# yuliangguo/OmniFusion

Measured on AMD Instinct MI355X. Metric: panoramas/sec at 512x1024 ERP, N=18 256^2 patches; equi2pers+pers2equi GB/s vs HBM peak, higher is better.
Workload: dtype f16x3 (fp16 hi/lo pairs, fp32 accumulate: fp32-class); 1 GPU; cfg2/cfg4 shard: 8 panoramas/GPU/step, 512x1024 ERP, fov 80, nrows 4 (18 patches); full single-pass spherical_fusion forward (confidence=True) at patch size 128 — the only size the reference network exists at (SURVEY 0.1); random-init weights (seed 42); inputs resident in HBM; resample pair at 18x256^2 reported in roofline_resample; per_gpu_batch=8, global_batch=8, parallelism=image-sharded x1, execution=3 forwards in flight per GPU on 3 streams (spherical_fusion.pipelined)

## Files before the change

### include/omnifusion.h

```cpp
#ifndef OMNIFUSION_H_
#define OMNIFUSION_H_

#include <stddef.h>
#include <stdint.h>

#ifdef __cplusplus
extern "C" {
#endif

#define OMNI_VERSION 200

enum omni_status {
    OMNI_OK = 0,
    OMNI_ERR_INVALID = 1,
    OMNI_ERR_HIP = 2,
    OMNI_ERR_UNSUPPORTED = 3
};

enum omni_layout { OMNI_LAYOUT_BCHWN = 0, OMNI_LAYOUT_BNCHW = 1, OMNI_LAYOUT_BNHWC = 2,
                   OMNI_LAYOUT_BCHNW = 3  };
enum omni_dtype { OMNI_F32 = 0, OMNI_F16 = 1 };

typedef void* omni_stream_t;
typedef struct omni_geometry omni_geometry_t;
// ... 61 lines not shown
int omni_gemm_rows_sh_f16x3(const void* x, const void* wt16r, const float* bias, const float* res, void* dst, int fmt,
                            int rows, int K, int N, int act, omni_stream_t stream);
int omni_gemm_rows_pack(const void* wt16, void* wt16r, int N, int K, omni_stream_t stream);
int omni_gemm_rows_ln_sh_f16x3(const float* x, const float* ln_weight, const float* ln_bias, float eps, const void* wt16r, const float* bias,
                               const float* res, void* dst, int fmt, int rows, int N, int act, omni_stream_t stream);
int omni_conv3x3_up2_sh_f16x3(const void* src, const void* wt16, const float* bias, void* dst, int fmt,
                              int M, int Hl, int Wl, int C, int Cout, int act, omni_stream_t stream);
size_t omni_up2_heads_scratch_bytes(int M, int P);
int omni_conv3x3_up2_heads_sh_f16x3(const void* src, const void* wt16, const float* bias, const void* heads_w16f, float bias_pred, float bias_weight,
                                    float* scratch, size_t scratch_bytes, float* out_a, float* out_c, int M, int P, int confidence, omni_stream_t stream);
int omni_conv3x3_up2_heads_sh_f16x1(const void* src, const void* wt16, const float* bias, const void* heads_w16f, float bias_pred, float bias_weight,
                                    float* scratch, size_t scratch_bytes, float* out_a, float* out_c, int M, int P, int confidence, omni_stream_t stream);
int omni_heads_pack_f16x3(const float* w_host, void* dst_host);
int omni_conv2d_sh_f16x3_post_ws(const void* src1, const void* src2, const void* wt16, const float* bias,
                                 const void* res, void* dst, int fmt, int M, int H, int W, int C1, int C2, int Cout,
                                 int KH, int KW, int stride, int pad, int act, int splitk, float* ws, size_t ws_bytes,
                                 const float* post, size_t post_elems, omni_stream_t stream);
int omni_wino_input_sh(const void* src, void* V, int M, int H, int W, int C, omni_stream_t stream);
int omni_conv3x3_wino_sh_f16x3(const void* V, const void* wt16, const float* bias, const void* res, void* dst, int fmt,
                               int M, int H, int W, int C, int Cout, int act, int splitk, float* ws, size_t ws_bytes, omni_stream_t stream);
int omni_sh_from_f32(const float* src, void* dst, size_t n, omni_stream_t stream);
int omni_sh_to_f32(const void* src, float* dst, size_t n, omni_stream_t stream);
int omni_sh_overflow(int* flag, int reset);
int omni_stem_f32(const float* src, const float* wt, const float* bias, float* dst, int M, int P, omni_stream_t stream);
int omni_maxpool3x3s2_f32(const float* src, float* dst, int M, int H, int W, int C, omni_stream_t stream);
int omni_upsample_bilinear_f32(const float* src, float* dst, int M, int H, int W, int C, int Ho, int Wo, omni_stream_t stream);
int omni_add_hw_f32(float* x, const float* y, int M, int HW, int C, omni_stream_t stream);
int omni_add_period_f32(float* x, const float* y, size_t total, size_t period, omni_stream_t stream);
int omni_stem_sh(const float* src, const float* wt, const float* bias, void* dst, int M, int P, omni_stream_t stream);
int omni_stem_sh_f16x3(const float* src, const void* wt16, const float* bias, void* dst, int M, int P, omni_stream_t stream);
int omni_stem_sh_f16x1(const float* src, const void* wt16, const float* bias, void* dst, int M, int P, omni_stream_t stream);
int omni_maxpool3x3s2_sh(const void* src, void* dst, int M, int H, int W, int C, omni_stream_t stream);
int omni_upsample_bilinear_sh(const void* src, void* dst, int M, int H, int W, int C, int Ho, int Wo, omni_stream_t stream);
int omni_add_hw_sh(void* x, const float* y, int M, int HW, int C, omni_stream_t stream);
int omni_add_period_sh(void* x, const float* y, size_t total, size_t period, omni_stream_t stream);
int omni_layernorm512_sh(const float* x, const float* g, const float* b, void* y, int rows, float eps, omni_stream_t stream);
int omni_gemm_rows_slices_sh_f16x3(const void* x, const void* wt16r, float* parts, int rows, int K, int N, int slices, omni_stream_t stream);
int omni_gemm_rows_ln_parts_sh_f16x3(const float* parts, int nparts, const float* pbias, const float* pres, float* xout,
                                     const float* ln_weight, const float* ln_bias, float eps, const void* wt16r, const float* bias,
                                     void* dst, int fmt, int rows, int N, int act, omni_stream_t stream);
int omni_splitk_reduce_ln512(const float* parts, int nparts, const float* bias, const float* res, float* tok, const float* ln_weight, const float* ln_bias,
                             float eps, void* y, int fmt, int rows, omni_stream_t stream);
int omni_gemm_sh_f16x3_ln512_ws(const void* x, const void* wt16, const float* bias, const float* res, float* tok, const float* ln_g, const float* ln_b,
                                float eps, void* y, int fmt, int rows, int K, int splitk, float* ws, size_t ws_bytes, omni_stream_t stream);
int omni_attention_qkv_sh(const float* qkv, void* out, int B, int N, omni_stream_t stream);
int omni_token_pack_f32(const float* d, const float* pos, float* tok, int M, int N, int HW, int C, omni_stream_t stream);
int omni_layernorm512_f32(const float* x, const float* g, const float* b, float* y, int rows, float eps, omni_stream_t stream);
int omni_attention_f32(const float* q, const float* kv, float* out, int B, int N, omni_stream_t stream);
int omni_heads_f32(const float* x, const float* w, float bias_pred, float bias_weight, float* out_a, float* out_c,
                   int M, int P, int confidence, omni_stream_t stream);
int omni_mlp_points_f32(const float* xyz, const float* depth, const float* w1, const float* b1, const float* w2,
                        const float* b2, float* out, int Mo, int N, int HW, omni_stream_t stream);

int omni_masked_median_f32(const float* x, const float* mask, size_t n, unsigned* ws, float* out, omni_stream_t stream);
int omni_depth_metrics_f32(float* pred, const float* gt, const float* mask, const float* scale_num, const float* scale_den,
                           size_t n, double* ws, float* out, omni_stream_t stream);

size_t omni_semantic_workspace_bytes(size_t npix);
int omni_semantic_step_f32(const float* logits, const int64_t* target, int B, int C, size_t HW, int64_t ignore_index, int K,
                           void* workspace, float* loss, int64_t* pred, int64_t* confusion, omni_stream_t stream);
int omni_semantic_grad_f32(const float* logits, const int64_t* target, int B, int C, size_t HW, int64_t ignore_index,
                           const void* workspace, const float* grad_out, float* grad_logits, omni_stream_t stream);
int omni_confusion_matrix_i64(const int64_t* pred, const int64_t* gt, size_t n, int K, int64_t* confusion, int64_t* n_bad,
                              omni_stream_t stream);

int omni_preprocess_rgb_u8(const unsigned char* src_hwc, float* dst_chw, int B, int Hs, int Ws, int H, int W, omni_stream_t stream);
// ... 67 lines not shown
```

### omnifusion_amd/_lib.py

```python
import ctypes
import os

_HERE = os.path.dirname(os.path.abspath(__file__))
LIB_PATH = os.environ.get("OMNI_LIB_VARIANT") or os.path.join(_HERE, "csrc", "libomnifusion_hip.so")
LIB_PATH_DEBUG = os.path.join(_HERE, "csrc", "libomnifusion_hip_dbg.so")

OMNI_OK, OMNI_ERR_INVALID, OMNI_ERR_HIP, OMNI_ERR_UNSUPPORTED = 0, 1, 2, 3
LAYOUT_BCHWN, LAYOUT_BNCHW, LAYOUT_BNHWC, LAYOUT_BCHNW = 0, 1, 2, 3
F32, F16 = 0, 1

_lib = None


class OmniLibraryMissing(ImportError):
    pass


EXPORTS = [
    "omni_version", "omni_last_error", "omni_set_option", "omni_get_option", "omni_num_patches", "omni_patch_centers",
    "omni_geometry_create", "omni_geometry_destroy", "omni_geometry_cache_clear", "omni_geometry_cache_size",
    "omni_equi2pers", "omni_equi2pers_aux", "omni_pers2equi", "omni_pers2equi_conf", "omni_patches_to_planar",
    "omni_equi2pers_g", "omni_pers2equi_g", "omni_equi2pers_bwd", "omni_pers2equi_bwd",
    "omni_conv2d_nhwc_f32", "omni_stem_f32", "omni_maxpool3x3s2_f32", "omni_upsample_bilinear_f32",
    "omni_add_hw_f32", "omni_add_period_f32", "omni_token_pack_f32", "omni_layernorm512_f32",
    "omni_attention_f32", "omni_heads_f32", "omni_mlp_points_f32",
    "omni_conv2d_nhwc_f16x3_ws", "omni_conv2d_sh_f16x3_ws", "omni_conv2d_sh_f16x3_post_ws", "omni_gemm_rows_sh_f16x3", "omni_gemm_rows_ln_sh_f16x3", "omni_gemm_rows_pack", "omni_conv3x3_up2_sh_f16x3", "omni_conv3x3_up2_heads_sh_f16x3", "omni_conv3x3_up2_heads_sh_f16x1", "omni_up2_heads_scratch_bytes", "omni_heads_pack_f16x3", "omni_sh_from_f32", "omni_sh_to_f32", "omni_sh_overflow",
    "omni_stem_sh", "omni_stem_sh_f16x3", "omni_stem_sh_f16x1", "omni_maxpool3x3s2_sh", "omni_upsample_bilinear_sh", "omni_add_hw_sh", "omni_add_period_sh", "omni_layernorm512_sh", "omni_gemm_sh_f16x3_ln512_ws", "omni_gemm_rows_slices_sh_f16x3", "omni_gemm_rows_ln_parts_sh_f16x3", "omni_splitk_reduce_ln512", "omni_wino_input_sh", "omni_conv3x3_wino_sh_f16x3", "omni_attention_qkv_sh",
    "omni_conv2d_splitk_plan", "omni_conv2d_nhwc_f32_ws",
    "omni_masked_median_f32", "omni_depth_metrics_f32",
    "omni_png_info", "omni_png_decode", "omni_png_decode_batch", "omni_zlib_inflate", "omni_png_checksums",
    "omni_preprocess_rgb_u8", "omni_preprocess_depth_u16", "omni_berhu_workspace_bytes", "omni_berhu_loss_f32", "omni_berhu_grad_f32",
    "omni_pointcloud_ply_f32",
    "omni_dibr_workspace_bytes", "omni_splat_render_f32", "omni_dibr_f32",
    "omni_splat_render_wt_f32", "omni_dibr_wt_f32", "omni_dibr_bwd_workspace_bytes", "omni_splat_render_bwd_f32", "omni_dibr_bwd_f32",
    "omni_ssim_f32", "omni_photometric_workspace_bytes", "omni_photometric_grad_scratch_bytes", "omni_photometric_loss_f32",
    "omni_photometric_grad_f32",
    "omni_freeview_rotations", "omni_freeview_equi2pers_f32", "omni_freeview_pers2equi_f32", "omni_freeview_merge_f32",
    "omni_freeview_bwd_workspace_bytes", "omni_freeview_equi2pers_bwd_f32", "omni_freeview_pers2equi_bwd_f32", "omni_freeview_merge_bwd_f32",
    "omni_semantic_workspace_bytes", "omni_semantic_step_f32", "omni_semantic_grad_f32", "omni_confusion_matrix_i64",
]


def load():
    global _lib
    if _lib is not None:
        return _lib
    if not os.path.exists(LIB_PATH):
        raise OmniLibraryMissing(
            f"{LIB_PATH} not found: build it with `python -m omnifusion_amd.build` "
            "(hipcc --offload-arch=gfx950).  There is no fallback path.")
    import torch
    lib = ctypes.CDLL(LIB_PATH)
    lib.omni_last_error.restype = ctypes.c_char_p
    lib.omni_version.restype = ctypes.c_int
    lib.omni_up2_heads_scratch_bytes.restype = ctypes.c_size_t
    lib.omni_dibr_workspace_bytes.restype = ctypes.c_size_t
    lib.omni_splat_render_f32.argtypes = [ctypes.c_void_p] * 3 + [ctypes.c_float] + [ctypes.c_void_p] * 2 + [ctypes.c_int] * 4 + [ctypes.c_void_p] * 2
    lib.omni_dibr_f32.argtypes = [ctypes.c_void_p] * 4 + [ctypes.c_int, ctypes.c_float, ctypes.c_int] + [ctypes.c_void_p] * 2 + \
        [ctypes.c_int] * 4 + [ctypes.c_void_p] * 2
    vp, ci, cf = ctypes.c_void_p, ctypes.c_int, ctypes.c_float
# ... 83 lines not shown
```

### omnifusion_amd/csrc/omni_net.hip

```cpp
#include "omni_internal.h"
#include "omni_sh.h"

namespace {
typedef float f4v __attribute__((ext_vector_type(4)));

template <bool SH>
__global__ __launch_bounds__(256) void stem_kernel(const float* __restrict__ src, const float* __restrict__ wt,
                                                   const float* __restrict__ bias, void* __restrict__ dst,
                                                   int M, int P, int Po)
{
    __shared__ __attribute__((aligned(16))) float wl[147 * 64];
    __shared__ float in[3][21][22];
    const int t = threadIdx.x;
    const int tiles = Po / 8;
    const int m = blockIdx.x / (tiles * tiles), tt = blockIdx.x % (tiles * tiles);
    const int oy0 = (tt / tiles) * 8, ox0 = (tt % tiles) * 8;
    for (int i = t; i < 147 * 64 / 4; i += 256) reinterpret_cast<f4v*>(wl)[i] = reinterpret_cast<const f4v*>(wt)[i];
    const int iy0 = oy0 * 2 - 3, ix0 = ox0 * 2 - 3;
    for (int i = t; i < 3 * 21 * 21; i += 256) {
        const int c = i / 441, r = (i % 441) / 21, q = i % 21;
        const int iy = iy0 + r, ix = ix0 + q;
        float v = 0.0f;
        if ((unsigned)iy < (unsigned)P && (unsigned)ix < (unsigned)P) v = src[((size_t)m * 3 + c) * P * P + (size_t)iy * P + ix];
        in[c][r][q] = v;
    }
    __syncthreads();
    const int p = t & 63, cg = (t >> 6) * 16;
    const int py = p >> 3, px = p & 7;
    float acc[16];
#pragma unroll
    for (int j = 0; j < 16; ++j) acc[j] = bias[cg + j];
    for (int ky = 0; ky < 7; ++ky)
// ... 81 lines not shown
    const int c8 = C / 8;
    const size_t total = (size_t)M * Ho * Wo * c8;
    if (i >= total) return;
    const int c = (int)(i % c8) * 8;
    size_t r = i / c8;
    const int ox = (int)(r % Wo); r /= Wo;
    const int oy = (int)(r % Ho); const int m = (int)(r / Ho);
    const float fy = fmaxf(sy * ((float)oy + 0.5f) - 0.5f, 0.0f), fx = fmaxf(sx * ((float)ox + 0.5f) - 0.5f, 0.0f);
    const int y0 = (int)fy, x0 = (int)fx;
    const int y1 = y0 + (y0 < H - 1 ? 1 : 0), x1 = x0 + (x0 < W - 1 ? 1 : 0);
    const float ly = fy - (float)y0, lx = fx - (float)x0, hy = 1.0f - ly, hx = 1.0f - lx;
    const size_t coff = (size_t)(c >> 5) * 128 + (c & 31) * 2;
    const size_t pp = (size_t)C * 4;
    const unsigned char* b = src + (size_t)m * H * W * pp + coff;
    const unsigned char* p00 = b + ((size_t)y0 * W + x0) * pp; const unsigned char* p01 = b + ((size_t)y0 * W + x1) * pp;
    const unsigned char* p10 = b + ((size_t)y1 * W + x0) * pp; const unsigned char* p11 = b + ((size_t)y1 * W + x1) * pp;
    const omni_h8v h00 = *reinterpret_cast<const omni_h8v*>(p00), l00 = *reinterpret_cast<const omni_h8v*>(p00 + 64);
    const omni_h8v h01 = *reinterpret_cast<const omni_h8v*>(p01), l01 = *reinterpret_cast<const omni_h8v*>(p01 + 64);
    const omni_h8v h10 = *reinterpret_cast<const omni_h8v*>(p10), l10 = *reinterpret_cast<const omni_h8v*>(p10 + 64);
    const omni_h8v h11 = *reinterpret_cast<const omni_h8v*>(p11), l11 = *reinterpret_cast<const omni_h8v*>(p11 + 64);
    omni_h8v oh, ol;
#pragma unroll
    for (int e = 0; e < 8; ++e) {
        const float v00 = fmaf((float)l00[e], 4.8828125e-4f, (float)h00[e]), v01 = fmaf((float)l01[e], 4.8828125e-4f, (float)h01[e]);
        const float v10 = fmaf((float)l10[e], 4.8828125e-4f, (float)h10[e]), v11 = fmaf((float)l11[e], 4.8828125e-4f, (float)h11[e]);
        const float o = hy * (hx * v00 + lx * v01) + ly * (hx * v10 + lx * v11);
        const _Float16 h = (fabsf(o) < 6.103515625e-05f) ? (_Float16)0.0f : (_Float16)o;
        oh[e] = h; ol[e] = (_Float16)((o - (float)h) * 2048.0f);
    }
    unsigned char* d = dst + (((size_t)m * Ho + oy) * Wo + ox) * pp + coff;
    *reinterpret_cast<omni_h8v*>(d) = oh; *reinterpret_cast<omni_h8v*>(d + 64) = ol;
}

__global__ __launch_bounds__(256) void add_hw_kernel(float* __restrict__ x, const float* __restrict__ y, size_t total, int HW, int C)
{
    const size_t i = (size_t)blockIdx.x * 256 + threadIdx.x;
    if (i >= total) return;
    const int c = (int)(i % C);
    const size_t m = i / ((size_t)HW * C);
    x[i] += y[m * C + c];
}
__global__ __launch_bounds__(256) void add_period_kernel(float* __restrict__ x, const float* __restrict__ y, size_t total, size_t period)
{
    const size_t i = (size_t)blockIdx.x * 256 + threadIdx.x;
    if (i >= total) return;
    x[i] += y[i % period];
}

__global__ __launch_bounds__(256) void add_hw_sh_kernel(void* __restrict__ x, const float* __restrict__ y, size_t total4, int HW, int C)
{
    const size_t i = (size_t)blockIdx.x * 256 + threadIdx.x;
    if (i >= total4) return;
    const size_t e = i * 4;
    const int c = (int)(e % C);
    const size_t m = e / ((size_t)HW * C);
    act_store4<true>(x, e, act_load4<true>(x, e) + *reinterpret_cast<const f4v*>(y + m * C + c));
}
__global__ __launch_bounds__(256) void add_period_sh_kernel(void* __restrict__ x, const float* __restrict__ y, size_t total4, size_t period)
{
    const size_t i = (size_t)blockIdx.x * 256 + threadIdx.x;
    if (i >= total4) return;
    const size_t e = i * 4;
    act_store4<true>(x, e, act_load4<true>(x, e) + *reinterpret_cast<const f4v*>(y + e % period));
}
__global__ __launch_bounds__(256) void token_pack_kernel(const float* __restrict__ d, const float* __restrict__ pos,
                                                         float* __restrict__ tok, int M, int N, int HW, int C)
// ... 201 lines not shown
}
int omni_add_hw_f32(float* x, const float* y, int M, int HW, int C, omni_stream_t stream)
{
    const size_t total = (size_t)M * HW * C;
    hipLaunchKernelGGL(add_hw_kernel, dim3(nblk(total)), dim3(256), 0, S_, x, y, total, HW, C);
    OMNI_HIP(hipGetLastError()); return OMNI_OK;
}
int omni_add_period_f32(float* x, const float* y, size_t total, size_t period, omni_stream_t stream)
{
    hipLaunchKernelGGL(add_period_kernel, dim3(nblk(total)), dim3(256), 0, S_, x, y, total, period);
    OMNI_HIP(hipGetLastError()); return OMNI_OK;
}
int omni_stem_sh(const float* src, const float* wt, const float* bias, void* dst, int M, int P, omni_stream_t stream)
{
    if (P % 16) OMNI_FAIL(OMNI_ERR_INVALID, "omni_stem: patch size must be a multiple of 16");
    const int Po = P / 2;
    hipLaunchKernelGGL(stem_kernel<true>, dim3(M * (Po / 8) * (Po / 8)), dim3(256), 0, S_, src, wt, bias, dst, M, P, Po);
    OMNI_HIP(hipGetLastError()); return OMNI_OK;
}
int omni_maxpool3x3s2_sh(const void* src, void* dst, int M, int H, int W, int C, omni_stream_t stream)
{
    if (C % 32) OMNI_FAIL(OMNI_ERR_INVALID, "SH tensors need C % 32 == 0");
    const int Ho = (H + 2 - 3) / 2 + 1, Wo = (W + 2 - 3) / 2 + 1;
    hipLaunchKernelGGL(maxpool_kernel<true>, dim3(nblk((size_t)M * Ho * Wo * C / 4)), dim3(256), 0, S_, src, dst, M, H, W, C, Ho, Wo);
    OMNI_HIP(hipGetLastError()); return OMNI_OK;
}
int omni_upsample_bilinear_sh(const void* src, void* dst, int M, int H, int W, int C, int Ho, int Wo, omni_stream_t stream)
{
    if (C % 32) OMNI_FAIL(OMNI_ERR_INVALID, "SH tensors need C % 32 == 0");
    hipLaunchKernelGGL(upsample_sh8_kernel, dim3(nblk((size_t)M * Ho * Wo * C / 8)), dim3(256), 0, S_, (const unsigned char*)src,
                       (unsigned char*)dst, M, H, W, C, Ho, Wo, (float)H / (float)Ho, (float)W / (float)Wo);
    OMNI_HIP(hipGetLastError()); return OMNI_OK;
}
int omni_add_hw_sh(void* x, const float* y, int M, int HW, int C, omni_stream_t stream)
{
    if (C % 32) OMNI_FAIL(OMNI_ERR_INVALID, "SH tensors need C % 32 == 0");
    const size_t total4 = (size_t)M * HW * C / 4;
    hipLaunchKernelGGL(add_hw_sh_kernel, dim3(nblk(total4)), dim3(256), 0, S_, x, y, total4, HW, C);
    OMNI_HIP(hipGetLastError()); return OMNI_OK;
}
int omni_add_period_sh(void* x, const float* y, size_t total, size_t period, omni_stream_t stream)
{
    if (total % 32 || period % 32) OMNI_FAIL(OMNI_ERR_INVALID, "SH tensors need C % 32 == 0");
    hipLaunchKernelGGL(add_period_sh_kernel, dim3(nblk(total / 4)), dim3(256), 0, S_, x, y, total / 4, period);
    OMNI_HIP(hipGetLastError()); return OMNI_OK;
}
int omni_layernorm512_sh(const float* x, const float* g, const float* b, void* y, int rows, float eps, omni_stream_t stream)
{
    hipLaunchKernelGGL(layernorm512_kernel<true>, dim3((rows + 3) / 4), dim3(256), 0, S_, x, g, b, y, rows, eps);
    OMNI_HIP(hipGetLastError()); return OMNI_OK;
}
int omni_attention_qkv_sh(const float* qkv, void* out, int B, int N, omni_stream_t stream)
{
    if (N > 64) OMNI_FAIL(OMNI_ERR_UNSUPPORTED, "omni_attention: at most 64 tokens");
    hipLaunchKernelGGL(attention_kernel<true>, dim3(B * 4, (N + 3) / 4), dim3(256), 0, S_, qkv, qkv + 512, out, N, 0.08838834764831845f, 1536, 1536, 512);
    OMNI_HIP(hipGetLastError()); return OMNI_OK;
}
int omni_token_pack_f32(const float* d, const float* pos, float* tok, int M, int N, int HW, int C, omni_stream_t stream)
{
    hipLaunchKernelGGL(token_pack_kernel, dim3(nblk((size_t)M * HW * C)), dim3(256), 0, S_, d, pos, tok, M, N, HW, C);
    OMNI_HIP(hipGetLastError()); return OMNI_OK;
}
int omni_layernorm512_f32(const float* x, const float* g, const float* b, float* y, int rows, float eps, omni_stream_t stream)
{
    hipLaunchKernelGGL(layernorm512_kernel<false>, dim3((rows + 3) / 4), dim3(256), 0, S_, x, g, b, (void*)y, rows, eps);
    OMNI_HIP(hipGetLastError()); return OMNI_OK;
// ... 23 lines not shown
```

### omnifusion_amd/model/_engine.py

```python
import ctypes
import os

import torch

from .. import _lib
from ..equi_pers.equi2pers_v3 import equi2pers_patches, equi2pers_aux, pair, _NPATCH
from ..equi_pers.pers2equi_v3 import pers2equi, pers2equi_conf

ACT_NONE, ACT_RELU, ACT_GELU = 0, 1, 2
_LAYERS = [("layer1", 3, 1), ("layer2", 4, 2), ("layer3", 6, 2), ("layer4", 3, 2)]
_BN_EPS = 1e-5
PRECISIONS = ("f16x3", "f16x1", "fp32")


def _p(t):
    return ctypes.c_void_p(t.data_ptr()) if t is not None else None


def split_weights_f16x3(w):
    w = w.to(torch.float32)
    wmax = float(w.abs().max()) if w.numel() else 0.0
    if not wmax < 65504.0:
        raise ValueError(f"folded weight magnitude {wmax:g} is outside the fp16 range of the f16x3 operand format: "
                         "run this checkpoint with OMNI_NET_PRECISION=fp32")
# ... 44 lines not shown
        g = sd[bn + ".weight"].double() / torch.sqrt(sd[bn + ".running_var"].double() + _BN_EPS)
        b = sd[bn + ".bias"].double() - sd[bn + ".running_mean"].double() * g
        return w * g[:, None, None, None], b

    @staticmethod
    def _gemm_layout(w):
        return w.permute(0, 2, 3, 1).reshape(w.shape[0], -1)

    def pack(self, state_dict, device):
        sd = {k: v.detach().cpu() for k, v in strip_module_prefix(state_dict).items()}
        dev = torch.device(device)
        f = lambda t: t.to(torch.float32).contiguous().to(dev)
        W = {}
        w, b = self._fold(sd, "conv1", "bn1")
        W["stem.w"] = f(w.permute(2, 3, 1, 0).reshape(147, 64)); W["stem.b"] = f(b)
        wk = torch.zeros((64, 3, 7, 8), dtype=torch.float64); wk[..., :7] = w
        W["stem.w16"] = split_weights_f16x3(torch.cat([wk.reshape(64, 168), torch.zeros((64, 24), dtype=torch.float64)], 1)).to(dev)

        def convbn(key, conv, bn):
            w, b = self._fold(sd, conv, bn)
            wg = self._gemm_layout(w).to(torch.float32)
            W[key + ".w"] = f(wg); W[key + ".b"] = f(b)
            W[key + ".w16"] = split_weights_f16x3(wg).to(dev)
        for lname, nblk, _ in _LAYERS:
            for i in range(nblk):
                p = f"{lname}.{i}"
                convbn(p + ".c1", p + ".conv1", p + ".bn1")
                convbn(p + ".c2", p + ".conv2", p + ".bn2")
                if (p + ".downsample.0.weight") in sd:
                    convbn(p + ".ds", p + ".downsample.0", p + ".downsample.1")
        for name in ("de_conv0_0", "de_conv0_1", "de_conv1_0", "de_conv1_1", "de_conv2_0", "de_conv2_1",
                     "de_conv3_0", "de_conv3_1", "de_conv4_0"):
            convbn(name, name + ".conv", name + ".bn")
        down = "down1" if self.iterative else "down"
        W["down.w"] = f(sd[down + ".weight"].reshape(32, 512)); W["down.b"] = f(sd[down + ".bias"])
        W["down.w16"] = split_weights_f16x3(sd[down + ".weight"].reshape(32, 512)).to(dev)
        W["pos"] = f(sd["transformer.pos_emb"].reshape(self.npatches, 512))
        for i in range(6):
            p = f"transformer.layer.{i}"
            for k in ("norm1.weight", "norm1.bias", "norm2.weight", "norm2.bias", "attn.q.weight", "attn.kv.weight",
                      "attn.proj.weight", "attn.proj.bias", "mlp.fc1.weight", "mlp.fc1.bias", "mlp.fc2.weight", "mlp.fc2.bias"):
                W[f"t{i}.{k}"] = f(sd[f"{p}.{k}"])
        for i in range(6):
            t = f"t{i}."
            W[t + "attn.qkv.w16"] = split_weights_f16x3(torch.cat([W[t + "attn.q.weight"], W[t + "attn.kv.weight"]], 0).cpu()).to(dev)
            for k in ("attn.proj", "mlp.fc1", "mlp.fc2"):
                W[t + k + ".w16"] = split_weights_f16x3(W[t + k + ".weight"].cpu()).to(dev)
        W["enc_norm.w"] = f(sd["transformer.encoder_norm.weight"]); W["enc_norm.b"] = f(sd["transformer.encoder_norm.bias"])
        hw = torch.stack([sd["pred.weight"][0, :, :, :, 0], sd["weight_pred.weight"][0, :, :, :, 0]])
        W["heads.w"] = f(hw.permute(0, 2, 3, 1).reshape(2, 9, 32))
        import numpy as np
        hw_host = np.ascontiguousarray(hw.permute(0, 2, 3, 1).reshape(2, 9, 32).to(torch.float32).numpy())
        frag = np.zeros(4 * 64 * 8, np.float16)
        _lib.check(_lib.load().omni_heads_pack_f16x3(hw_host.ctypes.data_as(ctypes.c_void_p), frag.ctypes.data_as(ctypes.c_void_p)), "heads_pack")
        W["heads.w16f"] = torch.from_numpy(frag).to(dev)
        self.head_bias = (float(sd["pred.bias"][0]), float(sd["weight_pred.bias"][0]))

        def mlp(name):
            w1, b1 = self._fold(sd, name + ".0", name + ".1")
            w2, b2 = self._fold(sd, name + ".3", name + ".4")
            return w1[:, :, 0, 0], b1, w2[:, :, 0, 0], b2
        P4 = self.patch_size[0] // 4
        if self.iterative:
            for name in ("mlp_points1", "mlp_points2"):
                w1, b1, w2, b2 = mlp(name)
                W[name + ".w1"], W[name + ".b1"], W[name + ".w2"], W[name + ".b2"] = f(w1), f(b1), f(w2), f(b2)
# ... 145 lines not shown
                                                      _p(self.w[bkey]) if bkey else None, None, _p(out), 1 if out_sh else 0, rows, Nout, act, self._s), "ln+gemm " + w16key)
            return out
        return self._gemm_sh(self._ln_sh(x, lnw, lnb, rows, eps), w16key, bkey, rows, 512, Nout, act=act, out_sh=out_sh)

    def _ln_sh(self, x, wk, bk, rows, eps):
        y = torch.empty_like(x)
        _lib.check(_lib.load().omni_layernorm512_sh(_p(x), _p(self.w[wk]), _p(self.w[bk]), _p(y), rows, ctypes.c_float(eps), self._s), "layernorm")
        return y

    def _ln(self, x, wk, bk, rows, eps):
        y = torch.empty_like(x)
        _lib.check(_lib.load().omni_layernorm512_f32(_p(x), _p(self.w[wk]), _p(self.w[bk]), _p(y), rows, ctypes.c_float(eps), self._s), "layernorm")
        return y

    def _up(self, x, M, H, Wd, C, Ho, Wo):
        y = torch.empty((M, Ho, Wo, C), dtype=torch.float32, device=x.device)
        fn = _lib.load().omni_upsample_bilinear_sh if self.sh else _lib.load().omni_upsample_bilinear_f32
        _lib.check(fn(_p(x), _p(y), M, H, Wd, C, Ho, Wo, self._s), "upsample")
        return y

    fold_point_feat = True
    fuse_up = True

    def _up_conv(self, x, key, M, H, Wd, C, Cout, act, out_f32=False, out=None):
        Ho, Wo = 2 * H, 2 * Wd
        if self.sh and self.fuse_up and Wo % 32 == 0 and Ho % 4 == 0:
            if out is None:
                out = torch.empty((M, Ho, Wo, Cout), dtype=torch.float32, device=x.device)
            _lib.check(_lib.load().omni_conv3x3_up2_sh_f16x3(_p(x), _p(self.w[key + ".w16"]), _p(self.w[key + ".b"]), _p(out),
                                                             (0 if out_f32 else 1) | (4 if (self._bs == 1 and self.latency_plan) else 0) | self._x1,
                                                             M, H, Wd, C, Cout, act, self._s), "up+conv " + key)
            return out
        return self._conv(self._up(x, M, H, Wd, C, Ho, Wo), key, M, Ho, Wo, C, Cout, 3, 1, 1, act, out_f32=out_f32, out=out)

    def transformer(self, d, bs):
        lib = _lib.load()
        dev = d.device
        self._s = ctypes.c_void_p(torch.cuda.current_stream(dev).cuda_stream)
        self._bs = bs
        N, P32 = self.npatches, self.patch_size[0] // 32
        M = bs * N
        sh = self.sh
        new = lambda *s: torch.empty(s, dtype=torch.float32, device=dev)
        tok = new(M, 512)
        _lib.check(lib.omni_token_pack_f32(_p(d), _p(self.w["pos"]), _p(tok), M, N, P32 * P32, 32, self._s), "token_pack")
        normed = None
        pending = None
        for i in range(6):
            t = f"t{i}."
            if sh:
                if pending is not None:
                    tok, qkv = self._ln_gemm_parts(pending, t + "norm1.weight", t + "norm1.bias", 1e-5, t + "attn.qkv.w16", M, 1536)
                    pending = None
                elif normed is not None:
                    qkv = self._gemm_sh(normed, t + "attn.qkv.w16", None, M, 512, 1536)
                else:
                    qkv = self._ln_gemm_sh(tok, t + "norm1.weight", t + "norm1.bias", 1e-5, t + "attn.qkv.w16", None, M, 1536)
                att = new(M, 512)
                _lib.check(lib.omni_attention_qkv_sh(_p(qkv), _p(att), bs, N, self._s), "attention")
                tok = self._gemm_sh(att, t + "attn.proj.w16", t + "attn.proj.bias", M, 512, 512, res=tok)
                h = self._ln_gemm_sh(tok, t + "norm2.weight", t + "norm2.bias", 1e-5, t + "mlp.fc1.w16", t + "mlp.fc1.bias", M, 2048, act=ACT_GELU, out_sh=True)
                nxt = (f"t{i + 1}.norm1.weight", f"t{i + 1}.norm1.bias", 1e-5, True) if i < 5 else ("enc_norm.w", "enc_norm.b", 1e-6, False)
                tok, normed, pending = self._fc2_ln(h, t + "mlp.fc2.w16", t + "mlp.fc2.bias", M, tok, nxt)
                continue
            y = self._ln(tok, t + "norm1.weight", t + "norm1.bias", M, 1e-5)
            q = self._gemm(y, t + "attn.q.weight", None, M, 512, 512)
# ... 32 lines not shown
                raise ValueError(f"precision f16x1 needs a patch size that is a multiple of 32 (got {P})")
            if sh and P % 32 == 0:
                _lib.check((lib.omni_stem_sh_f16x1 if self._x1 else lib.omni_stem_sh_f16x3)(_p(pat[m0:m1]), _p(self.w["stem.w16"]), _p(self.w["stem.b"]), _p(conv1[m0:m1]), Mc, P, self._s), "stem")
            else:
                _lib.check((lib.omni_stem_sh if sh else lib.omni_stem_f32)(_p(pat[m0:m1]), _p(self.w["stem.w"]), _p(self.w["stem.b"]),
                                                                            _p(conv1[m0:m1]), Mc, P, self._s), "stem")
            _lib.check((lib.omni_maxpool3x3s2_sh if sh else lib.omni_maxpool3x3s2_f32)(_p(conv1[m0:m1]), _p(x[m0:m1]), Mc, P2, P2, 64, self._s), "maxpool")
        feats = {}
        cin, size = 64, P4
        for lname, nblk, stride in _LAYERS:
            cout = {"layer1": 64, "layer2": 128, "layer3": 256, "layer4": 512}[lname]
            for i in range(nblk):
                p = f"{lname}.{i}"
                s = stride if i == 0 else 1
                ident = x
                if (p + ".ds.w") in self.w:
                    ident = self._conv(x, p + ".ds", M, size, size, cin, cout, 1, s, 0, ACT_NONE)
                y = self._conv(x, p + ".c1", M, size, size, cin, cout, 3, s, 1, ACT_RELU)
                size = (size + 2 - 3) // s + 1
                fold = sh and self.fold_point_feat and lname == "layer1" and i == nblk - 1
                x = self._conv(y, p + ".c2", M, size, size, cout, cout, 3, 1, 1, ACT_RELU, res=ident, post=point_feat if fold else None)
                cin = cout
            if lname == "layer1" and not (sh and self.fold_point_feat):
                _lib.check((lib.omni_add_period_sh if sh else lib.omni_add_period_f32)(
                    _p(x), _p(point_feat), ctypes.c_size_t(x.numel()), ctypes.c_size_t(point_feat.numel()), self._s), "add point_feat")
            feats[lname] = x
        layer1, layer2, layer3, layer4 = (feats[k] for k in ("layer1", "layer2", "layer3", "layer4"))
        if 32 * P32 * P32 != 512:
            raise RuntimeError(f"patch size {P}: token dim {32 * P32 * P32} != 512 — the reference network only exists at "
                               "patch size 128 (SURVEY.md finding 0.1)")
        d = self._conv(layer4, "down", M, P32, P32, 512, 32, 1, 1, 0, ACT_NONE, out_f32=True)
        tok = self.transformer(d, bs)
        _lib.check((lib.omni_add_hw_sh if sh else lib.omni_add_hw_f32)(_p(layer4), _p(tok), M, P32 * P32, 512, self._s), "token bias")
        up = self._up(layer4, M, P32, P32, 512, P16, P16)
        x = self._conv(up, "de_conv0_0", M, P16, P16, 512, 256, 3, 1, 1, ACT_RELU)
        x = self._conv(x, "de_conv0_1", M, P16, P16, 256, 128, 3, 1, 1, ACT_RELU, x2=layer3, C2=256)
        up = self._up(x, M, P16, P16, 128, P8, P8)
        x = self._conv(up, "de_conv1_0", M, P8, P8, 128, 128, 3, 1, 1, ACT_RELU)
        x = self._conv(x, "de_conv1_1", M, P8, P8, 128, 64, 3, 1, 1, ACT_RELU, x2=layer2, C2=128)
        x = self._up_conv(x, "de_conv2_0", M, P8, P8, 64, 64, ACT_RELU)
        x = self._conv(x, "de_conv2_1", M, P4, P4, 64, 64, 3, 1, 1, ACT_RELU, x2=layer1, C2=64)
        a, c = out if out is not None else (new(bs, N, 1, P, P), new(bs, N, 1, P, P) if confidence else None)
        av, cv = a.view(M, P, P), c.view(M, P, P) if c is not None else None
        fused = sh and self.fuse_heads and P % 32 == 0
        x_in, de4 = x, (None if fused else new(M, P, P, 32))
        for m0, m1 in self._chunks(bs, N, self.tail_chunk):
            Mc = m1 - m0
            x = self._up_conv(x_in[m0:m1], "de_conv3_0", Mc, P4, P4, 64, 64, ACT_RELU)
            x = self._conv(x, "de_conv3_1", Mc, P2, P2, 64, 32, 3, 1, 1, ACT_RELU, x2=conv1[m0:m1], C2=64)
            if fused:
                nb = int(lib.omni_up2_heads_scratch_bytes(Mc, P))
                hs = new((nb + 3) // 4)
                _lib.check((lib.omni_conv3x3_up2_heads_sh_f16x1 if self._x1 else lib.omni_conv3x3_up2_heads_sh_f16x3)(_p(x), _p(self.w["de_conv4_0.w16"]), _p(self.w["de_conv4_0.b"]), _p(self.w["heads.w16f"]),
                                                               ctypes.c_float(self.head_bias[0]), ctypes.c_float(self.head_bias[1]), _p(hs), ctypes.c_size_t(nb),
                                                               _p(av[m0:m1]), _p(cv[m0:m1]) if cv is not None else None, Mc, P, 1 if confidence else 0, self._s), "up+conv+heads")
                continue
            self._up_conv(x, "de_conv4_0", Mc, P2, P2, 32, 32, ACT_RELU, out_f32=True, out=de4[m0:m1])
            _lib.check(lib.omni_heads_f32(_p(de4[m0:m1]), _p(self.w["heads.w"]), ctypes.c_float(self.head_bias[0]), ctypes.c_float(self.head_bias[1]),
                                          _p(av[m0:m1]), _p(cv[m0:m1]) if cv is not None else None, Mc, P, 1 if confidence else 0, self._s), "heads")
        self.last = {"de_conv4_0": de4, "layer4": layer4}
        return a, c

    fuse_heads = os.environ.get("OMNI_FUSE_HEADS", "1") != "0"

    tail_chunk = 0
    front_chunk = 0

    @staticmethod
    def _chunks(bs, N, per):
        per = bs if per <= 0 else min(per, bs)
        return [(b0 * N, min(bs, b0 + per) * N) for b0 in range(0, bs, per)]
# ... 27 lines not shown
```

Measured before the change: 4093 panoramas/s.

## Reorder upsample and 3x3 conv as low-res tap GEMM plus bilinear tap-sum

For de_conv0_0, bilinear 2x upsampling followed by a 3x3 conv is replaced by an equivalent form. A 1x1 GEMM at low resolution produces all 9 per-tap outputs (9*Cout channels, fp32). A new kernel then bilinearly samples and sums those taps in LDS, adding bias and ReLU. This cuts the conv work by roughly the upsample area factor, since the GEMM runs on 4x4 instead of 8x8 pixels. The cost is an extra fp32 intermediate, a new kernel launch and a different rounding order. Weights for de_conv1_0 are prepared too, but only de_conv0_0 takes the new path.

```diff
diff --git a/include/omnifusion.h b/include/omnifusion.h
--- a/include/omnifusion.h
+++ b/include/omnifusion.h
@@ -117,6 +117,7 @@
 int omni_stem_sh_f16x1(const float* src, const void* wt16, const float* bias, void* dst, int M, int P, omni_stream_t stream);
 int omni_maxpool3x3s2_sh(const void* src, void* dst, int M, int H, int W, int C, omni_stream_t stream);
 int omni_upsample_bilinear_sh(const void* src, void* dst, int M, int H, int W, int C, int Ho, int Wo, omni_stream_t stream);
+int omni_up2_tapsum_sh(const float* y, const float* bias, void* dst, int M, int Hl, int Wl, int Cout, int act, omni_stream_t stream);
 int omni_add_hw_sh(void* x, const float* y, int M, int HW, int C, omni_stream_t stream);
 int omni_add_period_sh(void* x, const float* y, size_t total, size_t period, omni_stream_t stream);
 int omni_layernorm512_sh(const float* x, const float* g, const float* b, void* y, int rows, float eps, omni_stream_t stream);
diff --git a/omnifusion_amd/_lib.py b/omnifusion_amd/_lib.py
--- a/omnifusion_amd/_lib.py
+++ b/omnifusion_amd/_lib.py
@@ -25,7 +25,7 @@
     "omni_add_hw_f32", "omni_add_period_f32", "omni_token_pack_f32", "omni_layernorm512_f32",
     "omni_attention_f32", "omni_heads_f32", "omni_mlp_points_f32",
     "omni_conv2d_nhwc_f16x3_ws", "omni_conv2d_sh_f16x3_ws", "omni_conv2d_sh_f16x3_post_ws", "omni_gemm_rows_sh_f16x3", "omni_gemm_rows_ln_sh_f16x3", "omni_gemm_rows_pack", "omni_conv3x3_up2_sh_f16x3", "omni_conv3x3_up2_heads_sh_f16x3", "omni_conv3x3_up2_heads_sh_f16x1", "omni_up2_heads_scratch_bytes", "omni_heads_pack_f16x3", "omni_sh_from_f32", "omni_sh_to_f32", "omni_sh_overflow",
-    "omni_stem_sh", "omni_stem_sh_f16x3", "omni_stem_sh_f16x1", "omni_maxpool3x3s2_sh", "omni_upsample_bilinear_sh", "omni_add_hw_sh", "omni_add_period_sh", "omni_layernorm512_sh", "omni_gemm_sh_f16x3_ln512_ws", "omni_gemm_rows_slices_sh_f16x3", "omni_gemm_rows_ln_parts_sh_f16x3", "omni_splitk_reduce_ln512", "omni_wino_input_sh", "omni_conv3x3_wino_sh_f16x3", "omni_attention_qkv_sh",
+    "omni_stem_sh", "omni_stem_sh_f16x3", "omni_stem_sh_f16x1", "omni_maxpool3x3s2_sh", "omni_upsample_bilinear_sh", "omni_up2_tapsum_sh", "omni_add_hw_sh", "omni_add_period_sh", "omni_layernorm512_sh", "omni_gemm_sh_f16x3_ln512_ws", "omni_gemm_rows_slices_sh_f16x3", "omni_gemm_rows_ln_parts_sh_f16x3", "omni_splitk_reduce_ln512", "omni_wino_input_sh", "omni_conv3x3_wino_sh_f16x3", "omni_attention_qkv_sh",
     "omni_conv2d_splitk_plan", "omni_conv2d_nhwc_f32_ws",
     "omni_masked_median_f32", "omni_depth_metrics_f32",
     "omni_png_info", "omni_png_decode", "omni_png_decode_batch", "omni_zlib_inflate", "omni_png_checksums",
diff --git a/omnifusion_amd/csrc/omni_net.hip b/omnifusion_amd/csrc/omni_net.hip
--- a/omnifusion_amd/csrc/omni_net.hip
+++ b/omnifusion_amd/csrc/omni_net.hip
@@ -1,3 +1,4 @@
+#include <algorithm>
 #include "omni_internal.h"
 #include "omni_sh.h"
 
@@ -145,6 +146,59 @@
     *reinterpret_cast<omni_h8v*>(d) = oh; *reinterpret_cast<omni_h8v*>(d + 64) = ol;
 }
 
+constexpr int TS_SLAB = 32, TS_PITCH = 9 * TS_SLAB, TS_MAX_HW = 64;
+__global__ __launch_bounds__(256) void up2_tapsum_sh_kernel(const float* __restrict__ y, const float* __restrict__ bias, void* __restrict__ dst,
+                                                            int Hl, int Wl, int Cout, int act)
+{
+    extern __shared__ __attribute__((aligned(16))) float ts_img[];
+    const int m = blockIdx.x, c0 = blockIdx.y * TS_SLAB, HW = Hl * Wl;
+    const float* src = y + (size_t)m * HW * 9 * Cout + c0;
+    const int nq = HW * 9 * (TS_SLAB / 4);
+#pragma unroll 4
+    for (int i = threadIdx.x; i < nq; i += 256)
+        *reinterpret_cast<f4v*>(ts_img + i * 4) = *reinterpret_cast<const f4v*>(src + (size_t)(i >> 3) * Cout + (i & 7) * 4);
+    __syncthreads();
+    const int Ho = 2 * Hl, Wo = 2 * Wl, NP = Ho * Wo;
+    const int lane = threadIdx.x & 63, wave = threadIdx.x >> 6;
+    const int pi = ((lane >> 5) << 2) | ((0x31130220u >> (((lane >> 2) & 7) * 4)) & 3);
+    const int q = (lane & 7) * 4;
+    f4v bv = (f4v)(0.0f);
+    if (bias) bv = *reinterpret_cast<const f4v*>(bias + c0 + q);
+    for (int p = wave * 8 + pi; p < NP; p += 32) {
+        const int oy = p / Wo, ox = p - oy * Wo;
+        int yo0[3], yo1[3], xo0[3], xo1[3];
+        float ly[3], lx[3];
+        bool vy[3], vx[3];
+#pragma unroll
+        for (int k = 0; k < 3; ++k) {
+            const int py = oy + k - 1, px = ox + k - 1;
+            vy[k] = (unsigned)py < (unsigned)Ho; vx[k] = (unsigned)px < (unsigned)Wo;
+            const float fy = fmaxf(0.5f * ((float)py + 0.5f) - 0.5f, 0.0f), fx = fmaxf(0.5f * ((float)px + 0.5f) - 0.5f, 0.0f);
+            const int y0 = (int)fy, x0 = (int)fx;
+            ly[k] = fy - (float)y0; lx[k] = fx - (float)x0;
+            yo0[k] = y0 * Wl * TS_PITCH; yo1[k] = (y0 + (y0 < Hl - 1 ? 1 : 0)) * Wl * TS_PITCH;
+            xo0[k] = x0 * TS_PITCH;      xo1[k] = (x0 + (x0 < Wl - 1 ? 1 : 0)) * TS_PITCH;
+        }
+        f4v acc = (f4v)(0.0f);
+#pragma unroll
+        for (int ky = 0; ky < 3; ++ky)
+#pragma unroll
+            for (int kx = 0; kx < 3; ++kx) {
+                if (!(vy[ky] && vx[kx])) continue;
+                const float* b = ts_img + (ky * 3 + kx) * TS_SLAB + q;
+                const f4v v00 = *reinterpret_cast<const f4v*>(b + yo0[ky] + xo0[kx]), v01 = *reinterpret_cast<const f4v*>(b + yo0[ky] + xo1[kx]);
+                const f4v v10 = *reinterpret_cast<const f4v*>(b + yo1[ky] + xo0[kx]), v11 = *reinterpret_cast<const f4v*>(b + yo1[ky] + xo1[kx]);
+                const float hy = 1.0f - ly[ky], hx = 1.0f - lx[kx];
+                const float w00 = hy * hx, w01 = hy * lx[kx], w10 = ly[ky] * hx, w11 = ly[ky] * lx[kx];
+#pragma unroll
+                for (int e = 0; e < 4; ++e) acc[e] = fmaf(w11, v11[e], fmaf(w10, v10[e], fmaf(w01, v01[e], fmaf(w00, v00[e], acc[e]))));
+            }
+        f4v o = acc + bv;
+        if (act == OMNI_ACT_RELU) { o.x = fmaxf(o.x, 0.f); o.y = fmaxf(o.y, 0.f); o.z = fmaxf(o.z, 0.f); o.w = fmaxf(o.w, 0.f); }
+        act_store4<true>(dst, (((size_t)m * Ho + oy) * Wo + ox) * Cout + c0 + q, o);
+    }
+}
+
 __global__ __launch_bounds__(256) void add_hw_kernel(float* __restrict__ x, const float* __restrict__ y, size_t total, int HW, int C)
 {
     const size_t i = (size_t)blockIdx.x * 256 + threadIdx.x;
@@ -412,6 +466,27 @@
                        (unsigned char*)dst, M, H, W, C, Ho, Wo, (float)H / (float)Ho, (float)W / (float)Wo);
     OMNI_HIP(hipGetLastError()); return OMNI_OK;
 }
+int omni_up2_tapsum_sh(const float* y, const float* bias, void* dst, int M, int Hl, int Wl, int Cout, int act, omni_stream_t stream)
+{
+    if (!y || !dst || M < 1 || Hl < 1 || Wl < 1 || Cout < 1) OMNI_FAIL(OMNI_ERR_INVALID, "omni_up2_tapsum_sh: null tensor or empty shape");
+    if ((uintptr_t)y % 16 || (uintptr_t)bias % 16 || (uintptr_t)dst % 16) OMNI_FAIL(OMNI_ERR_INVALID, "omni_up2_tapsum_sh: tensors must be 16-byte aligned");
+    if (Cout % TS_SLAB || Cout / TS_SLAB > 65535 || (long long)Hl * Wl > TS_MAX_HW || (act != OMNI_ACT_NONE && act != OMNI_ACT_RELU))
+        OMNI_FAIL(OMNI_ERR_UNSUPPORTED, "omni_up2_tapsum_sh: Cout % 32 == 0, Hl * Wl <= 64, no activation or ReLU");
+    const size_t lds = (size_t)Hl * Wl * TS_PITCH * sizeof(float);
+    if (lds > 64 * 1024) {
+        static std::mutex mu;
+        static std::vector<int> done;
+        int dev = 0;
+        OMNI_HIP(hipGetDevice(&dev));
+        std::lock_guard<std::mutex> lk(mu);
+        if (std::find(done.begin(), done.end(), dev) == done.end()) {
+            OMNI_HIP(hipFuncSetAttribute(reinterpret_cast<const void*>(up2_tapsum_sh_kernel), hipFuncAttributeMaxDynamicSharedMemorySize, TS_MAX_HW * TS_PITCH * (int)sizeof(float)));
+            done.push_back(dev);
+        }
+    }
+    hipLaunchKernelGGL(up2_tapsum_sh_kernel, dim3((unsigned)M, (unsigned)(Cout / TS_SLAB)), dim3(256), lds, S_, y, bias, dst, Hl, Wl, Cout, act);
+    OMNI_HIP(hipGetLastError()); return OMNI_OK;
+}
 int omni_add_hw_sh(void* x, const float* y, int M, int HW, int C, omni_stream_t stream)
 {
     if (C % 32) OMNI_FAIL(OMNI_ERR_INVALID, "SH tensors need C % 32 == 0");
diff --git a/omnifusion_amd/model/_engine.py b/omnifusion_amd/model/_engine.py
--- a/omnifusion_amd/model/_engine.py
+++ b/omnifusion_amd/model/_engine.py
@@ -100,6 +100,9 @@
         for name in ("de_conv0_0", "de_conv0_1", "de_conv1_0", "de_conv1_1", "de_conv2_0", "de_conv2_1",
                      "de_conv3_0", "de_conv3_1", "de_conv4_0"):
             convbn(name, name + ".conv", name + ".bn")
+        for name in ("de_conv0_0", "de_conv1_0"):
+            w, _ = self._fold(sd, name + ".conv", name + ".bn")
+            W[name + ".taps.w16"] = split_weights_f16x3(w.permute(2, 3, 0, 1).reshape(9 * w.shape[0], w.shape[1]).to(torch.float32)).to(dev)
         down = "down1" if self.iterative else "down"
         W["down.w"] = f(sd[down + ".weight"].reshape(32, 512)); W["down.b"] = f(sd[down + ".bias"])
         W["down.w16"] = split_weights_f16x3(sd[down + ".weight"].reshape(32, 512)).to(dev)
@@ -311,6 +314,16 @@
                                                              M, H, Wd, C, Cout, act, self._s), "up+conv " + key)
             return out
         return self._conv(self._up(x, M, H, Wd, C, Ho, Wo), key, M, Ho, Wo, C, Cout, 3, 1, 1, act, out_f32=out_f32, out=out)
+
+    taps_first = frozenset(("de_conv0_0",))
+
+    def _up_conv_taps(self, x, key, M, H, Wd, C, Cout, act):
+        if key in self.taps_first and self.sh and self.terms == 3 and Cout % 32 == 0 and H * Wd <= 64:
+            y = self._conv(x, key + ".taps", M, H, Wd, C, 9 * Cout, 1, 1, 0, ACT_NONE, bias=False, out_f32=True)
+            out = torch.empty((M, 2 * H, 2 * Wd, Cout), dtype=torch.float32, device=x.device)
+            _lib.check(_lib.load().omni_up2_tapsum_sh(_p(y), _p(self.w[key + ".b"]), _p(out), M, H, Wd, Cout, act, self._s), "tap sum " + key)
+            return out
+        return self._conv(self._up(x, M, H, Wd, C, 2 * H, 2 * Wd), key, M, 2 * H, 2 * Wd, C, Cout, 3, 1, 1, act)
 
     def transformer(self, d, bs):
         lib = _lib.load()
@@ -409,11 +422,9 @@
         d = self._conv(layer4, "down", M, P32, P32, 512, 32, 1, 1, 0, ACT_NONE, out_f32=True)
         tok = self.transformer(d, bs)
         _lib.check((lib.omni_add_hw_sh if sh else lib.omni_add_hw_f32)(_p(layer4), _p(tok), M, P32 * P32, 512, self._s), "token bias")
-        up = self._up(layer4, M, P32, P32, 512, P16, P16)
-        x = self._conv(up, "de_conv0_0", M, P16, P16, 512, 256, 3, 1, 1, ACT_RELU)
+        x = self._up_conv_taps(layer4, "de_conv0_0", M, P32, P32, 512, 256, ACT_RELU)
         x = self._conv(x, "de_conv0_1", M, P16, P16, 256, 128, 3, 1, 1, ACT_RELU, x2=layer3, C2=256)
-        up = self._up(x, M, P16, P16, 128, P8, P8)
-        x = self._conv(up, "de_conv1_0", M, P8, P8, 128, 128, 3, 1, 1, ACT_RELU)
+        x = self._up_conv_taps(x, "de_conv1_0", M, P16, P16, 128, 128, ACT_RELU)
         x = self._conv(x, "de_conv1_1", M, P8, P8, 128, 64, 3, 1, 1, ACT_RELU, x2=layer2, C2=128)
         x = self._up_conv(x, "de_conv2_0", M, P8, P8, 64, 64, ACT_RELU)
         x = self._conv(x, "de_conv2_1", M, P4, P4, 64, 64, 3, 1, 1, ACT_RELU, x2=layer1, C2=64)
```

Measured after the change: 4174 panoramas/s, median of 6. 2.0% higher.
